# Virtana/accurate-aprilgroup-tracking

Hardware: AMD Instinct MI355X
Metric: frames/sec (LK+PnP) on 1280x720 dodeca stream (higher is better)
Workload: dtype u8/i64 (LK), f64 (PnP); 1 GPU; c2: 1 x 1280x720 stream(s) per GPU, 12 tags/48 corners, 3-level LK 21x21, iterative PnP with motion-model guess; streams_per_gpu=1, frames_resident=HBM ring 368 slots (323 MiB), parallelism=stream-per-GPU x1, RCCL all_gather of poses once per block

## Files before the change

### accurate_aprilgroup_tracking_amd/csrc/agt_pnp_body.h

```cpp
#pragma once
#include <type_traits>
#include <cstddef>
#include "agt_device.h"
#include "agt_kernels.h"

#ifdef AGT_PNP_STAMPS
__device__ unsigned long long agt_pnp_stamps[64];
#define PSTAMP(i) do { if (b == 0 && threadIdx.x == 0) agt_pnp_stamps[i] = __builtin_amdgcn_s_memtime(); } while (0)
#define PSTAMPM(i) do { int mk_; asm volatile("s_mov_b32 %0, %1" : "=s"(mk_) : "n"(0xbeef00 + (i))); PSTAMP(i); } while (0)
extern "C" int agt_debug_pnp_stamps(unsigned long long* host64)
{
    return (int)hipMemcpyFromSymbol(host64, HIP_SYMBOL(agt_pnp_stamps), sizeof(agt_pnp_stamps));
}
#else
#define PSTAMP(i)
#define PSTAMPM(i)
#endif

#pragma clang fp contract(fast)

namespace agt_pnp {

constexpr int NACC = 28;
constexpr int SLAB = 65;
constexpr int MAX_PPL = 4;

__device__ __forceinline__ void pnp_sync()
{
    __builtin_amdgcn_fence(__ATOMIC_RELEASE, "wavefront");
    __builtin_amdgcn_wave_barrier();
    __builtin_amdgcn_fence(__ATOMIC_ACQUIRE, "wavefront");
}

struct PnpShared {
    double part[NACC * SLAB];
    double tot[NACC + 4];
    double LL[144];
    double vec[48];
    unsigned long long tab[5 * AGT_MAX_GROUP];
    int seq;
    int late;
    int coop[2];
    AgtTrackState ts;
};

typedef __attribute__((address_space(3))) AgtTrackState AgtTrackStateLds;

template <int K, bool READBACK = true>
__device__ __forceinline__ void wave_reduce_slab(double (&vals)[K], PnpShared& sh, int lane)
{
    static_assert(K <= NACC, "the slab holds NACC rows");
    pnp_sync();
#pragma unroll
    for (int k = 0; k < K; k++) sh.part[k * SLAB + lane] = vals[k];
    pnp_sync();
    const int k = lane & 31, h = lane >> 5;
    double s = 0.0;
    if (k < K) {
        const double* p = &sh.part[k * SLAB + 32 * h];
#pragma unroll 8
        for (int i = 0; i < 32; i++) s += p[i];
    }
    s += __shfl_xor(s, 32);
    if (lane < K) sh.tot[lane] = s;
    pnp_sync();
    if (READBACK) {
#pragma unroll
        for (int i = 0; i < K; i++) vals[i] = sh.tot[i];
    }
}

__device__ __forceinline__ double dswap32(double a, double b, double& b_out)
{
    const auto lo = __builtin_amdgcn_permlane32_swap((unsigned)__double2loint(a), (unsigned)__double2loint(b), false, false);
    const auto hi = __builtin_amdgcn_permlane32_swap((unsigned)__double2hiint(a), (unsigned)__double2hiint(b), false, false);
    b_out = __hiloint2double((int)hi[1], (int)lo[1]);
    return __hiloint2double((int)hi[0], (int)lo[0]);
}
__device__ __forceinline__ double dswap16(double a, double b, double& b_out)
{
    const auto lo = __builtin_amdgcn_permlane16_swap((unsigned)__double2loint(a), (unsigned)__double2loint(b), false, false);
    const auto hi = __builtin_amdgcn_permlane16_swap((unsigned)__double2hiint(a), (unsigned)__double2hiint(b), false, false);
    b_out = __hiloint2double((int)hi[1], (int)lo[1]);
    return __hiloint2double((int)hi[0], (int)lo[0]);
}
template <int CTRL>
__device__ __forceinline__ double ddpp(double v)
{
    return __hiloint2double(agt_dpp_i32<CTRL>(__double2hiint(v)), agt_dpp_i32<CTRL>(__double2loint(v)));
}
template <int CTRL, int N>
__device__ __forceinline__ void bfly_stage(double (&v)[32], bool upper)
{
#pragma unroll
    for (int i = 0; i < N; i++) {
        const double a = v[i], b = v[i + N];
        const double keep = upper ? b : a, send = upper ? a : b;
// ... 255 lines not shown
        }
        const int slot = n_after - 1;
        for (int i = 0; i < 9; i++) ts->rot_vel[slot][i] = rot_vel[i];
        for (int i = 0; i < 3; i++) ts->tran_vel[slot][i] = tran_vel[i];
        ts->n_vel = n_after;
    }
    if (n_after < 2) return 0;
    double dv[3], tran_acc[3], rot_acc[9];
#pragma unroll
    for (int i = 0; i < 3; i++) dv[i] = old_tv[i] - tran_vel[i];
    mat3_tvec(rot_vel, dv, tran_acc);
    mat3_tmul(rot_vel, old_rv, rot_acc);
    const double sy = agt_sqrtp(rot_acc[0] * rot_acc[0] + rot_acc[3] * rot_acc[3]);
    const bool sing = sy < 1e-6;
    double ay, ax;
    if (lane == 0) { ay = sing ? -rot_acc[5] : rot_acc[7]; ax = sing ? rot_acc[4] : rot_acc[8]; }
    else if (lane == 1) { ay = -rot_acc[6]; ax = sy; }
    else { ay = sing ? 0.0 : rot_acc[3]; ax = sing ? 1.0 : rot_acc[0]; }
    double sn, cs;
    {
        const double r = agt_sqrtp(ax * ax + ay * ay);
        if (r > 0.0) {
            const double ir = agt_rcp(r), c = ax * ir, sv = ay * ir;
            if (c >= 0.0) { cs = agt_sqrtp(0.5 * (1.0 + c)); sn = sv * agt_rcp(2.0 * cs); }
            else { const double a = agt_sqrtp(0.5 * (1.0 - c)); sn = copysign(a, ay); cs = fabs(sv) * agt_rcp(2.0 * a); }
        } else { cs = 1.0; sn = 0.0; }
    }
    const double sx = lane_bcast(sn, 0), cx = lane_bcast(cs, 0);
    const double sy2 = lane_bcast(sn, 1), cy = lane_bcast(cs, 1);
    const double sz = lane_bcast(sn, 2), cz = lane_bcast(cs, 2);
    const double Rx[9] = { 1, 0, 0, 0, cx, -sx, 0, sx, cx };
    const double Ry[9] = { cy, 0, sy2, 0, 1, 0, -sy2, 0, cy };
    const double Rz[9] = { cz, -sz, 0, sz, cz, 0, 0, 0, 1 };
    double Tm[9], RA[9], M[9], Rpred[9], tp[3], tpred[3];
    agt_mat3_mul(Ry, Rx, Tm);
    agt_mat3_mul(Rz, Tm, RA);
    agt_mat3_mul(RA, rot_vel, M);
    agt_mat3_mul(M, Rp, Rpred);
#pragma unroll
    for (int i = 0; i < 3; i++) tp[i] = prev[3 + i];
#pragma unroll
    for (int i = 0; i < 3; i++)
        tpred[i] = (M[i * 3] * tp[0] + M[i * 3 + 1] * tp[1] + M[i * 3 + 2] * tp[2]) +
                   (RA[i * 3] * tran_vel[0] + RA[i * 3 + 1] * tran_vel[1] + RA[i * 3 + 2] * tran_vel[2] + 0.5 * tran_acc[i]);
    double rpred[3];
    agt_rodrigues_inv(Rpred, rpred);
    if (lane == 0) {
        for (int i = 0; i < 3; i++) { ts->guess[i] = rpred[i]; ts->guess[3 + i] = (double)(float)tpred[i]; }
        ts->guess_t_f32 = 1;
    }
    return 0;
}

struct PnpNoHook { __device__ __forceinline__ void operator()() const {} };

template <typename T, int PPL, typename Hook = PnpNoHook, bool LDS_STATE = false, int COOP = 1, bool OPAQUE = false, bool VIS = false, bool CONS = false>
__device__ __forceinline__ void pnp_body(const AgtPnpParams& P, int b, PnpShared& sh, const void* img_p, const uint8_t* mask_p,
                                         double* so_p, int extra_flags = 0, Hook before_state = Hook())
{
    using TS = typename std::conditional<LDS_STATE, AgtTrackStateLds, AgtTrackState>::type;
    static_assert(COOP == 1 || (PPL == 1 && COOP * 32 * 3 <= NACC * SLAB), "cooperating waves hold one point per lane; slabs live in sh.part");
    int tid_ = (int)threadIdx.x;
    if constexpr (OPAQUE) asm volatile("" : "+v"(tid_));
    const int lane = tid_ & (AGT_WAVE - 1);
    const int wave = COOP > 1 ? agt_uniform(tid_ >> 6) : 0;
    const bool master = wave == 0;
    const bool writer = lane == 0 && master;
    const int n = P.n;
    int slab_sel = 0;
    double* const tot = COOP > 1 ? &sh.part[2 * COOP * 32 + wave * 32] : sh.tot;
    auto coop_sum = [&](double v) -> double {
        if constexpr (COOP == 1) return v;
        else {
            double* slot = &sh.part[slab_sel * COOP * 32];
            if (lane == 0) slot[wave * 32] = v;
            __syncthreads();
            double s_ = slot[0];
#pragma unroll
            for (int w = 1; w < COOP; w++) s_ += slot[w * 32];
            slab_sel ^= 1;
            return s_;
        }
    };
    PSTAMP(0);
    AgtCamera cam;
    load_cam<T>(P.cam, cam);

    double X[PPL], Y[PPL], Z[PPL], mu_[PPL], mv_[PPL];
    bool use[PPL];
    const int hyp_T = CONS ? P.hyp_T : 0;
    const int hs = hyp_T ? b / hyp_T : b;
    const T* obj = reinterpret_cast<const T*>(P.obj) + (long)hs * P.obj_bstride + (hyp_T ? (long)(b - hs * hyp_T) * n * 3 : 0L);
    const T* img = reinterpret_cast<const T*>(img_p) + (long)b * n * 2;
    const uint8_t* mask = mask_p ? mask_p + (long)b * n : nullptr;
    const uint8_t* cons = (CONS && P.cons_inl) ? P.cons_inl + (long)b * n : nullptr;
    int cnt = 0;
#pragma unroll
    for (int q = 0; q < PPL; q++) {
        const int i = lane + (q * COOP + wave) * AGT_WAVE;
        use[q] = i < n && (!mask || mask[i] != 0) && (!cons || cons[i] != 0);
        X[q] = Y[q] = Z[q] = mu_[q] = mv_[q] = 0.0;
        if (use[q]) {
            X[q] = (double)obj[i * 3]; Y[q] = (double)obj[i * 3 + 1]; Z[q] = (double)obj[i * 3 + 2];
            mu_[q] = (double)img[i * 2]; mv_[q] = (double)img[i * 2 + 1];
            cnt++;
        }
    }
    if (P.seed_pts) {
        for (int i = lane + wave * AGT_WAVE; i < n; i += AGT_WAVE * COOP) {
            P.seed_pts[((long)b * n + i) * 2] = (float)img[i * 2]; P.seed_pts[((long)b * n + i) * 2 + 1] = (float)img[i * 2 + 1];
            P.seed_status[(long)b * n + i] = (!mask || mask[i] != 0) ? 1 : 0;
        }
    }
    if (P.tag_gate) {
        cnt = 0;
#pragma unroll
        for (int q = 0; q < PPL; q++) {
            int u = use[q] ? 1 : 0;
            u &= agt_dpp_i32<0xB1>(u);
            u &= agt_dpp_i32<0x4E>(u);
            use[q] = u != 0;
            if (!use[q]) X[q] = Y[q] = Z[q] = mu_[q] = mv_[q] = 0.0;
            cnt += u;
        }
    }
    const int n_used = (int)coop_sum((double)agt_wave_sum_i64(cnt));
    before_state();
    int flags = extra_flags;
    double param[6];
    TS* ts;
    if constexpr (LDS_STATE) ts = (TS*)&sh.ts;
    else ts = P.track ? P.track + b : nullptr;
    if (ts && (agt_uniform(ts->chain_fault) | (extra_flags & AGT_TRK_CHAIN_TIMEOUT))) {
        if (writer) {
            ts->chain_fault = 1; ts->frame++;
            if (P.fault) __hip_atomic_store(P.fault, 1, __ATOMIC_RELAXED, __HIP_MEMORY_SCOPE_SYSTEM);
            if (P.dense_pose) {
                for (int i = 0; i < AGT_DENSE_STRIDE; i++) P.dense_rec[(long)b * AGT_DENSE_STRIDE + i] = 0.0;
                P.dense_done[b] = 1;
            }
            if (so_p) {
                double* so = so_p + (long)b * AGT_STATE_STRIDE;
                for (int i = 0; i < AGT_STATE_STRIDE; i++) so[i] = 0.0;
                so[AGT_ST_NTRACK] = n_used; so[AGT_ST_FLAGS] = AGT_TRK_CHAIN_TIMEOUT;
            }
        }
        return;
    }
    bool use_guess = P.use_guess != 0;
    double unchanged_prev[6] = { 0, 0, 0, 0, 0, 0 };
    int had_guess = 0, guess_f32 = 0, prev_f32 = 0;
    if (ts) {
        had_guess = ts->has_guess; guess_f32 = ts->guess_t_f32; prev_f32 = ts->prev_t_f32;
        use_guess = had_guess && P.enhance_ape;
#pragma unroll
        for (int i = 0; i < 6; i++) { unchanged_prev[i] = ts->prev[i]; param[i] = ts->guess[i]; }
        static_assert(offsetof(AgtTrackState, tran_vel) - offsetof(AgtTrackState, rot_vel) == 18 * sizeof(double) &&
                      offsetof(AgtTrackState, prev_R) - offsetof(AgtTrackState, rot_vel) == 24 * sizeof(double), "state layout");
        if (had_guess && P.enhance_ape && lane < 33 && master) sh.vec[lane] = (&ts->rot_vel[0][0])[lane];
        if (n_used < P.min_points) {
            if (writer) {
                ts->has_guess = 0; ts->frame++;
                if (P.dense_pose) {
                    for (int i = 0; i < AGT_DENSE_STRIDE; i++) P.dense_rec[(long)b * AGT_DENSE_STRIDE + i] = 0.0;
                    P.dense_done[b] = 1;
                }
                if (so_p) {
                    double* so = so_p + (long)b * AGT_STATE_STRIDE;
                    for (int i = 0; i < AGT_STATE_STRIDE; i++) so[i] = 0.0;
                    so[AGT_ST_NTRACK] = n_used; so[AGT_ST_FLAGS] = AGT_PNP_TOO_FEW | flags;
                    if constexpr (CONS) { if (P.cons_votes) so[AGT_ST_NINLIER] = (double)P.cons_votes[b * 4 + 1]; }
                    if constexpr (CONS) { if (P.pred_hist) so[AGT_ST_FLOW] = P.pred_hist[(long)b * AGT_PRED_STRIDE + AGT_PRED_FLOW]; }
                }
            }
            return;
        }
    } else {
        const double* start = P.pose + (long)b * 6;
        if constexpr (CONS) {
            if (P.hyp_track) { use_guess = agt_uniform(P.hyp_track[hs].has_guess) && P.enhance_ape; start = P.hyp_track[hs].guess; }
            else if (P.hyp_pose) start = P.hyp_pose + (long)hs * 6;
        }
#pragma unroll
        for (int i = 0; i < 6; i++) param[i] = start[i];
    }

    const bool enough = use_guess ? n_used >= 3 : n_used >= 4;
    if (!enough) {
        if (writer && P.info) {
            P.info[b * 4 + AGT_INFO_OK] = 0; P.info[b * 4 + AGT_INFO_ITERS] = 0;
            P.info[b * 4 + AGT_INFO_NUSED] = n_used; P.info[b * 4 + AGT_INFO_FLAGS] = AGT_PNP_TOO_FEW;
        }
        if (writer && P.err) P.err[b] = 0.0;
        return;
    }

    if constexpr (COOP > 1) { if (!use_guess) return; }
    if constexpr (COOP == 1) if (!use_guess) {
        double c4[4] = { 0, 0, 0, 0 };
#pragma unroll
        for (int q = 0; q < PPL; q++) if (use[q]) { c4[0] += X[q]; c4[1] += Y[q]; c4[2] += Z[q]; }
        wave_reduce_slab<4>(c4, sh, lane);
        const double mcx = c4[0] / n_used, mcy = c4[1] / n_used, mcz = c4[2] / n_used;
        double m6[6] = { 0, 0, 0, 0, 0, 0 };
#pragma unroll
        for (int q = 0; q < PPL; q++) if (use[q]) {
            const double dx = X[q] - mcx, dy = Y[q] - mcy, dz = Z[q] - mcz;
            m6[0] += dx * dx; m6[1] += dx * dy; m6[2] += dx * dz; m6[3] += dy * dy; m6[4] += dy * dz; m6[5] += dz * dz;
        }
        wave_reduce_slab<6>(m6, sh, lane);
        const double MM[9] = { m6[0], m6[1], m6[2], m6[1], m6[3], m6[4], m6[2], m6[4], m6[5] };
        double Wm[3], Um[9], Vm[9];
        agt_svd3(MM, Wm, Um, Vm);
        if (Wm[2] / Wm[1] < 1e-3) {
            flags |= AGT_PNP_PLANAR;
            double Rt[9];
#pragma unroll
            for (int i = 0; i < 9; i++) Rt[i] = Vm[i];
            if (Vm[2] * Vm[2] + Vm[5] * Vm[5] < 1e-10) {
#pragma unroll
                for (int i = 0; i < 9; i++) Rt[i] = (i % 4 == 0) ? 1.0 : 0.0;
            }
            if (agt_det3(Rt) < 0) {
#pragma unroll
                for (int i = 0; i < 9; i++) Rt[i] = -Rt[i];
            }
            double Tt[3];
#pragma unroll
            for (int a = 0; a < 3; a++) Tt[a] = -(Rt[a * 3] * mcx + Rt[a * 3 + 1] * mcy + Rt[a * 3 + 2] * mcz);
            double px_[PPL], py_[PPL], nx_[PPL], ny_[PPL];
            double c8[8] = { 0, 0, 0, 0, 0, 0, 0, 0 };
#pragma unroll
            for (int q = 0; q < PPL; q++) {
                px_[q] = py_[q] = nx_[q] = ny_[q] = 0.0;
                if (use[q]) {
                    px_[q] = (double)(float)(Rt[0] * X[q] + Rt[1] * Y[q] + Rt[2] * Z[q] + Tt[0]);
                    py_[q] = (double)(float)(Rt[3] * X[q] + Rt[4] * Y[q] + Rt[5] * Z[q] + Tt[1]);
                    undistort5(cam, mu_[q], mv_[q], nx_[q], ny_[q]);
                    nx_[q] = (double)(float)nx_[q]; ny_[q] = (double)(float)ny_[q];
                    c8[0] += nx_[q]; c8[1] += ny_[q]; c8[2] += px_[q]; c8[3] += py_[q];
                }
            }
            wave_reduce_slab<8>(c8, sh, lane);
            const double cmx = c8[0] / n_used, cmy = c8[1] / n_used, cMx = c8[2] / n_used, cMy = c8[3] / n_used;
            double d8[8] = { 0, 0, 0, 0, 0, 0, 0, 0 };
#pragma unroll
            for (int q = 0; q < PPL; q++) if (use[q]) {
                d8[0] += fabs(nx_[q] - cmx); d8[1] += fabs(ny_[q] - cmy); d8[2] += fabs(px_[q] - cMx); d8[3] += fabs(py_[q] - cMy);
            }
            wave_reduce_slab<8>(d8, sh, lane);
// ... 168 lines not shown
                            lambda_h = lc = 1.0 / sh.vec[14];
                            nu *= 0.5;
                        }
                        lambda_h *= nu;
                    }
                    if (Sd < S) {
#pragma unroll
                        for (int i = 0; i < 8; i++) hx[i] = xd[i];
                        hom_eval(hx);
                        rinf = rinf_d;
                    }
                    it++;
                    double dinf = 0.0;
#pragma unroll
                    for (int i = 0; i < 8; i++) dinf = fmax(dinf, fabs(dd[i]));
                    if (!(it < 10 && dinf >= (double)FLT_EPSILON && rinf >= (double)FLT_EPSILON)) break;
                }
            }
            pnp_sync();
            if (lane == 0) {
                double h[9];
                for (int i = 0; i < 8; i++) h[i] = hx[i];
                h[8] = sh.vec[40];
                double Rm[9], tv[3];
                if (h_ok) {
                    const double h1n = sqrt(h[0] * h[0] + h[3] * h[3] + h[6] * h[6]);
                    const double h2n = sqrt(h[1] * h[1] + h[4] * h[4] + h[7] * h[7]);
                    const double s1 = 1. / fmax(h1n, DBL_EPSILON), s2 = 1. / fmax(h2n, DBL_EPSILON), s3 = 2. / fmax(h1n + h2n, DBL_EPSILON);
                    const double t3[3] = { h[2] * s3, h[5] * s3, h[8] * s3 };
                    h[0] *= s1; h[3] *= s1; h[6] *= s1;
                    h[1] *= s2; h[4] *= s2; h[7] *= s2;
                    h[2] = h[3] * h[7] - h[6] * h[4];
                    h[5] = h[6] * h[1] - h[0] * h[7];
                    h[8] = h[0] * h[4] - h[3] * h[1];
                    double rr[3], dummy[27];
                    agt_rodrigues_inv(h, rr);
                    agt_rodrigues<false>(rr, h, dummy);
                    for (int a = 0; a < 3; a++) tv[a] = h[a * 3] * Tt[0] + h[a * 3 + 1] * Tt[1] + h[a * 3 + 2] * Tt[2] + t3[a];
                    agt_mat3_mul(h, Rt, Rm);
                } else {
                    for (int i = 0; i < 9; i++) Rm[i] = (i % 4 == 0) ? 1.0 : 0.0;
                    tv[0] = tv[1] = tv[2] = 0.0;
                }
                double rv[3];
                agt_rodrigues_inv(Rm, rv);
                sh.vec[32] = rv[0]; sh.vec[33] = rv[1]; sh.vec[34] = rv[2];
                sh.vec[35] = tv[0]; sh.vec[36] = tv[1]; sh.vec[37] = tv[2];
            }
            pnp_sync();
#pragma unroll
            for (int i = 0; i < 6; i++) param[i] = sh.vec[32 + i];
        } else {
        if (n_used < 6) {
            if (lane == 0 && P.info) {
                P.info[b * 4 + AGT_INFO_OK] = 0; P.info[b * 4 + AGT_INFO_ITERS] = 0;
                P.info[b * 4 + AGT_INFO_NUSED] = n_used; P.info[b * 4 + AGT_INFO_FLAGS] = AGT_PNP_TOO_FEW;
            }
            if (lane == 0 && P.err) P.err[b] = 0.0;
            if (lane == 0 && ts) {
                ts->has_guess = 0; ts->frame++;
                if (P.dense_pose) {
                    for (int i = 0; i < AGT_DENSE_STRIDE; i++) P.dense_rec[(long)b * AGT_DENSE_STRIDE + i] = 0.0;
                    P.dense_done[b] = 1;
                }
                if (so_p) {
                    double* so = so_p + (long)b * AGT_STATE_STRIDE;
                    for (int i = 0; i < AGT_STATE_STRIDE; i++) so[i] = 0.0;
                    so[AGT_ST_NTRACK] = n_used; so[AGT_ST_FLAGS] = AGT_PNP_TOO_FEW | flags;
                    if constexpr (CONS) { if (P.cons_votes) so[AGT_ST_NINLIER] = (double)P.cons_votes[b * 4 + 1]; }
                    if constexpr (CONS) { if (P.pred_hist) so[AGT_ST_FLOW] = P.pred_hist[(long)b * AGT_PRED_STRIDE + AGT_PRED_FLOW]; }
                }
            }
            return;
        }
        double s0[10], sx[10], sy[10], sq[10];
#pragma unroll
        for (int i = 0; i < 10; i++) s0[i] = sx[i] = sy[i] = sq[i] = 0.0;
#pragma unroll
        for (int q = 0; q < PPL; q++) if (use[q]) {
            double xn, yn;
            undistort5(cam, mu_[q], mv_[q], xn, yn);
            const double x = -xn, y = -yn, w2 = x * x + y * y;
            const double pr[10] = { X[q] * X[q], X[q] * Y[q], X[q] * Z[q], X[q], Y[q] * Y[q], Y[q] * Z[q], Y[q], Z[q] * Z[q], Z[q], 1.0 };
#pragma unroll
            for (int i = 0; i < 10; i++) { s0[i] += pr[i]; sx[i] += x * pr[i]; sy[i] += y * pr[i]; sq[i] += w2 * pr[i]; }
        }
        wave_reduce_slab<10>(s0, sh, lane);
        wave_reduce_slab<10>(sx, sh, lane);
        wave_reduce_slab<10>(sy, sh, lane);
        wave_reduce_slab<10>(sq, sh, lane);
        pnp_sync();
        if (lane == 0) {
            const int ui[4][4] = { { 0, 1, 2, 3 }, { 1, 4, 5, 6 }, { 2, 5, 7, 8 }, { 3, 6, 8, 9 } };
            for (int a = 0; a < 4; a++)
                for (int c = 0; c < 4; c++) {
                    const int u = ui[a][c];
                    sh.LL[a * 12 + c] = s0[u];           sh.LL[a * 12 + 4 + c] = 0.0;          sh.LL[a * 12 + 8 + c] = sx[u];
                    sh.LL[(4 + a) * 12 + c] = 0.0;       sh.LL[(4 + a) * 12 + 4 + c] = s0[u];  sh.LL[(4 + a) * 12 + 8 + c] = sy[u];
                    sh.LL[(8 + a) * 12 + c] = sx[u];     sh.LL[(8 + a) * 12 + 4 + c] = sy[u];  sh.LL[(8 + a) * 12 + 8 + c] = sq[u];
                }
        }
        pnp_sync();
        smallest_eigvec_wave<12>(sh.LL, sh.vec, lane);
        if (lane == 0) {
            double* v = sh.vec;
            double RR[9] = { v[0], v[1], v[2], v[4], v[5], v[6], v[8], v[9], v[10] };
            double tt[3] = { v[3], v[7], v[11] };
            if (agt_det3(RR) < 0) {
                for (int i = 0; i < 9; i++) RR[i] = -RR[i];
                for (int i = 0; i < 3; i++) tt[i] = -tt[i];
            }
            double sc = 0;
            for (int i = 0; i < 9; i++) sc += RR[i] * RR[i];
            sc = sqrt(sc);
            double Wr[3], U[9], Vt[9], Rm[9];
            agt_svd3(RR, Wr, U, Vt);
            agt_mat3_mul(U, Vt, Rm);
            double nr = 0;
            for (int i = 0; i < 9; i++) nr += Rm[i] * Rm[i];
            nr = sqrt(nr);
            double rv[3];
            agt_rodrigues_inv(Rm, rv);
            sh.vec[32] = rv[0]; sh.vec[33] = rv[1]; sh.vec[34] = rv[2];
            sh.vec[35] = tt[0] * nr / sc; sh.vec[36] = tt[1] * nr / sc; sh.vec[37] = tt[2] * nr / sc;
        }
        pnp_sync();
// ... 74 lines not shown
#pragma unroll
            for (int i = 0; i < 6; i++) JtErr[i] = tot[21 + i];
            return tot[27];
        }
        double e2 = 0.0;
#pragma unroll
        for (int q = 0; q < PPL; q++) if (PPL > 1 || use[q]) {
            double u, v;
            agt_project<false, D>(cam, R, G, param + 3, X[q], Y[q], Z[q], u, v, nullptr, nullptr);
            const double m = (PPL > 1 && !use[q]) ? 0.0 : 1.0;
            const double ex = (u - mu_[q]) * m, ey = (v - mv_[q]) * m;
            rex[q] = ex; rey[q] = ey;
            e2 += ex * ex + ey * ey;
        }
        return coop_sum(wave_sum_f64(e2));
    };
    auto evaluate = [&](int mode) -> double {
        return has_dist ? evaluate_t(mode, std::true_type{}) : evaluate_t(mode, std::false_type{});
    };
    auto commit_candidate = [&]() {
#pragma unroll
        for (int i = 0; i < 21; i++) JtJ[i] = tot[i];
#pragma unroll
        for (int i = 0; i < 6; i++) JtErr[i] = tot[21 + i];
    };
    auto residuals_same_rotation = [&](auto DIST) {
        constexpr bool D = decltype(DIST)::value;
#pragma unroll
        for (int q = 0; q < PPL; q++) if (use[q]) {
            double u, v;
            agt_project<false, D>(cam, Rlast, nullptr, param + 3, X[q], Y[q], Z[q], u, v, nullptr, nullptr);
            rex[q] = u - mu_[q]; rey[q] = v - mv_[q];
        }
    };

    auto step = [&]() {
        double A[36], dx[6];
        int idx = 0;
#pragma unroll
        for (int a = 0; a < 6; a++)
#pragma unroll
            for (int c = a; c < 6; c++) { A[a * 6 + c] = JtJ[idx]; A[c * 6 + a] = JtJ[idx]; idx++; }
#pragma unroll
        for (int a = 0; a < 6; a++) A[a * 7] *= 1.0 + lambda;
        if (!agt_solve6(A, JtErr, dx)) {
            flags |= AGT_PNP_SINGULAR;
#pragma unroll
            for (int a = 0; a < 6; a++) dx[a] = 0.0;
        }
#pragma unroll
        for (int a = 0; a < 6; a++) param[a] = prevParam[a] - dx[a];
    };

    PSTAMP(1);
    double e2 = evaluate(1);
    PSTAMP(2);
    for (;;) {
#pragma unroll
        for (int i = 0; i < 6; i++) prevParam[i] = param[i];
        if (iters == 0) prevErrNorm = sqrt(e2);
        double rel = 0.0, e2cand = 0.0;
        bool last = false;
        for (;;) {
            PSTAMP(8 + iters * 4 + 0);
            step();
            PSTAMP(8 + iters * 4 + 1);
            double dn = 0.0, pn = 0.0;
#pragma unroll
            for (int i = 0; i < 6; i++) { const double d = param[i] - prevParam[i]; dn += d * d; pn += prevParam[i] * prevParam[i]; }
            rel = sqrt(dn) / (sqrt(pn) + DBL_EPSILON);
            last = iters + 1 >= max_iter || rel < epsilon;
            e2cand = evaluate(last ? 0 : 2);
            errNorm = sqrt(e2cand);
            PSTAMP(8 + iters * 4 + 2);
            if (errNorm > prevErrNorm) { ++lambdaLg10; lambda *= 10.0; if (lambdaLg10 <= 16) continue; }
            break;
        }
        if (lambdaLg10 - 1 >= -16) { lambdaLg10 -= 1; lambda *= 0.1; } else { lambdaLg10 = -16; lambda = 1e-16; }
        ++iters;
        if (last) break;
        prevErrNorm = errNorm;
        commit_candidate();
        e2 = e2cand;
        PSTAMP(8 + (iters - 1) * 4 + 3);
    }
    PSTAMP(3);

    const bool tvec_f32 = ts && use_guess && guess_f32;
    if (tvec_f32) {
#pragma unroll
        for (int i = 3; i < 6; i++) param[i] = (double)(float)param[i];
    }

    double esum = 0.0;
    {
        if (tvec_f32) { if (has_dist) residuals_same_rotation(std::true_type{}); else residuals_same_rotation(std::false_type{}); }
#pragma unroll
        for (int q = 0; q < PPL; q++) if (use[q]) esum += sqrt(rex[q] * rex[q] + rey[q] * rey[q]);
        esum = coop_sum(wave_sum_f64(esum)) / n_used;
    }
    PSTAMP(4);
    if (!master) return;
    if (ts) {
        const bool accepted = esum < P.gate_px;
        int tflags = flags;
        if (writer && use_guess) {
            for (int i = 0; i < 6; i++) ts->guess[i] = param[i];
        }
        if (accepted && had_guess && P.enhance_ape)
            tflags |= motion_model_update(ts, lane, param, tvec_f32, unchanged_prev, prev_f32 != 0, Rlast, sh.vec);
        if (writer) {
            if (accepted) {
                if (!had_guess || !P.enhance_ape) {
                    for (int i = 0; i < 6; i++) ts->guess[i] = param[i];
                    ts->guess_t_f32 = 0; ts->has_guess = 1;
                }
                if (!(tflags & AGT_TRK_ZERO_VELOCITY)) {
                    for (int i = 0; i < 6; i++) ts->prev[i] = param[i];
                    for (int i = 0; i < 9; i++) ts->prev_R[i] = Rlast[i];
                    ts->prev_t_f32 = tvec_f32 ? 1 : 0; ts->has_prev = 1;
                }
            } else {
                ts->has_guess = 0;
            }
            ts->frame++;
            PSTAMP(5);
            if (P.dense_pose) {
                double* rc = P.dense_rec + (long)b * AGT_DENSE_STRIDE;
                for (int i = 0; i < 6; i++) { P.dense_pose[(long)b * 6 + i] = param[i]; rc[i] = param[i]; }
                for (int i = 6; i < AGT_DENSE_STRIDE; i++) rc[i] = 0.0;
                P.dense_done[b] = accepted ? 0 : 1;
            }
            if (so_p) {
                double* so = so_p + (long)b * AGT_STATE_STRIDE;
                for (int i = 0; i < 6; i++) so[i] = param[i];
                so[AGT_ST_OK] = accepted ? 1.0 : 0.0; so[AGT_ST_ERR] = esum; so[AGT_ST_NTRACK] = n_used;
                so[AGT_ST_ITERS] = iters; so[AGT_ST_GUESS] = use_guess ? 1.0 : 0.0; so[AGT_ST_FLAGS] = tflags;
                so[AGT_ST_TVEC_F32] = tvec_f32 ? 1.0 : 0.0;
                for (int i = AGT_ST_TVEC_F32 + 1; i < AGT_STATE_STRIDE; i++) so[i] = 0.0;
                if constexpr (CONS) { if (P.cons_votes) so[AGT_ST_NINLIER] = (double)P.cons_votes[b * 4 + 1]; }
                if constexpr (CONS) { if (P.pred_hist) so[AGT_ST_FLOW] = P.pred_hist[(long)b * AGT_PRED_STRIDE + AGT_PRED_FLOW]; }
            }
            if constexpr (CONS) {
                if (P.pred_hist) {
                    double* h = P.pred_hist + (long)b * AGT_PRED_STRIDE + AGT_PRED_LAST;
                    for (int i = 0; i < 6; i++) h[i] = param[i];
                    h[6] = accepted ? 1.0 : 0.0;
                }
            }
        }
        if (accepted && P.reproject && P.corners_rw) {
            double R[9], G[9];
            agt_rodrigues<false>(param, R, G);
            float* cw = P.corners_rw + (long)b * n * 2;
            const int cpt = VIS ? P.vis_cpt : 0;
            unsigned long long seen = ~0ull;
            if (cpt > 0) {
                double cs;
                const bool vis = lane < n / cpt && agt_tag_visible(obj + (long)lane * cpt * 3, cpt, R, param + 3, (double)P.vis_facing, P.vis_cos_max, cs);
                seen = __ballot(vis);
                if (writer && so_p) so_p[(long)b * AGT_STATE_STRIDE + AGT_ST_NVISIBLE] = (double)__popcll(seen);
            }
            for (int i = lane; i < n; i += AGT_WAVE) {
                double u, v;
                agt_project<false>(cam, R, G, param + 3, (double)obj[i * 3], (double)obj[i * 3 + 1], (double)obj[i * 3 + 2],
                                   u, v, nullptr, nullptr);
                cw[i * 2] = (float)u; cw[i * 2 + 1] = (float)v;
                if (P.status_rw) P.status_rw[(long)b * n + i] = cpt > 0 ? (uint8_t)((seen >> (i / cpt)) & 1) : 1;
            }
        }
        return;
    }
    if (writer) {
#pragma unroll
        for (int i = 0; i < 6; i++) P.pose[(long)b * 6 + i] = param[i];
        if (P.info) {
            P.info[b * 4 + AGT_INFO_OK] = 1; P.info[b * 4 + AGT_INFO_ITERS] = iters;
            P.info[b * 4 + AGT_INFO_NUSED] = n_used; P.info[b * 4 + AGT_INFO_FLAGS] = flags;
        }
        if (P.err) P.err[b] = esum;
    }
}

}

#pragma clang fp contract(off)
```

### accurate_aprilgroup_tracking_amd/csrc/agt_step.hip

```cpp
#undef AGT_LK_STAMPS
#undef AGT_PNP_STAMPS
#include "agt_step_args.h"
#include "agt_knobs.h"

#ifdef AGT_STEP_STAMPS
__device__ unsigned long long agt_step_stamps[16];
#define SSTAMP_SET(i) do { if (threadIdx.x == 0) agt_step_stamps[i] = __builtin_amdgcn_s_memtime(); } while (0)
#define SSTAMP_MAX(i) do { if (threadIdx.x == 0) atomicMax(&agt_step_stamps[i], (unsigned long long)__builtin_amdgcn_s_memtime()); } while (0)
#define SSTAMP_MIN(i) do { if (threadIdx.x == 0) atomicMin(&agt_step_stamps[i], (unsigned long long)__builtin_amdgcn_s_memtime()); } while (0)
extern "C" int agt_debug_step_stamps(unsigned long long* host16, int reset)
{
    int rc = (int)hipMemcpyFromSymbol(host16, HIP_SYMBOL(agt_step_stamps), sizeof(agt_step_stamps));
    if (reset) {
        unsigned long long z[16];
        for (int i = 0; i < 16; i++) z[i] = (i == 6) ? ~0ull : 0ull;
        rc |= (int)hipMemcpyToSymbol(HIP_SYMBOL(agt_step_stamps), z, sizeof(z));
    }
    return rc;
}
__device__ unsigned long long agt_role_stamps[AGT_MAX_GROUP * 4];
#define RSTAMP(k, i) do { if (blk == 0 && lane == 0) agt_role_stamps[(k) * 4 + (i)] = __builtin_amdgcn_s_memtime(); } while (0)
extern "C" int agt_debug_role_stamps(unsigned long long* host) { return (int)hipMemcpyFromSymbol(host, HIP_SYMBOL(agt_role_stamps), sizeof(agt_role_stamps)); }
#else
#define SSTAMP_SET(i)
#define SSTAMP_MAX(i)
#define SSTAMP_MIN(i)
#define RSTAMP(k, i)
#endif


typedef unsigned long long __attribute__((may_alias)) agt_word_t;
__device__ __forceinline__ void agt_copy_words_to_lds(void* dst_lds, const void* src, int n8, int t, int stride)
{
    for (int i = t; i < n8; i += stride) static_cast<agt_word_t*>(dst_lds)[i] = static_cast<const agt_word_t*>(src)[i];
}
typedef unsigned int __attribute__((may_alias)) agt_halfword_t;
__device__ __forceinline__ void agt_copy_halfwords_to_lds(void* dst_lds, const void* src, int n4, int t, int stride)
{
    for (int i = t; i < n4; i += stride) static_cast<agt_halfword_t*>(dst_lds)[i] = static_cast<const agt_halfword_t*>(src)[i];
}
__device__ __forceinline__ bool agt_ptr_plausible(unsigned long long p) { return (p >> 47) == 0; }
template <int NLEV>
__device__ __forceinline__ bool lk_table_bad(const agt_lk::LkFrameIo<NLEV>& io, int max_level)
{
    unsigned long long acc = (unsigned long long)io.next_pts | (unsigned long long)io.status | (unsigned long long)io.done;
    bool null_img = io.next_pts == nullptr || io.status == nullptr;
#pragma unroll
    for (int l = 0; l < NLEV; l++)
        if (l <= max_level) {
            acc |= (unsigned long long)io.imgI[l] | (unsigned long long)io.imgJ[l];
            null_img = null_img || io.imgI[l] == nullptr || io.imgJ[l] == nullptr;
        }
    return agt_uniform((int)(null_img || !agt_ptr_plausible(acc))) != 0;
}

hipError_t agt_launch_pnp_group_coop(hipStream_t stream, const AgtStepParams& P, const AgtStepTables& T);
hipError_t agt_launch_step_deep(hipStream_t stream, const AgtStepParams& P, const AgtStepTables& T, int blocks, size_t lds);

namespace {

template <int WIN, int NW, int NLEV, bool XCD_MAP = false>
__device__ __forceinline__ void lk_role(const AgtStepParams& S, const AgtStepTables& T, KParams KS, KTables KT, int blk, uint8_t* lds)
{
    static_assert(NW == 4, "one corner per workgroup of four waves");
    if constexpr (XCD_MAP) blk = agt_xcd_order(blk, (int)gridDim.x, KS->xshift);
    const long corner = blk;
    if (corner >= (long)S.lk.n * S.lk_B) return;
    const int b = (int)(corner / S.lk.n), pt = (int)(corner - (long)b * S.lk.n);
    constexpr size_t LKB = sizeof(AgtLkTables);
    const size_t per = lk_role_lds<WIN, NW, NLEV>(S.lk.max_level + 1);
    uint8_t* my = lds;
    AgtLkTables* tab = reinterpret_cast<AgtLkTables*>(my + per - LKB);
    {
        static_assert(sizeof(AgtLkTables) % 8 == 0, "table copy: 8-byte words");
        const int tid = (int)threadIdx.x;
        if (S.lk_nf > 1) agt_copy_words_to_lds(tab, (const void*)(const __attribute__((address_space(4))) void*)&KT->lk, (int)(LKB / 8), tid, AGT_WAVE * NW);
    }
    if constexpr (WIN == 21 && NW == 4) {
        if (S.lk.flags == 0 && S.lk.err == nullptr) {
            auto frame = [&](int k) {
// ... 39 lines not shown
        if (io.bad) return;
        agt_lk::lk_body<WIN, NW, NLEV>(&KS->lk, pt, b, my, io, px, py, pst);
    }
}

template <bool ROLL2>
__device__ __forceinline__ void pyr_role(KParams KS, KTables KT, int blk, int base, uint8_t* lds)
{
#pragma unroll
    for (int s = 0; s < AGT_MAX_LEVELS - 1; s++) {
        const int n = KS->n_pyr[s];
        if (blk < n) {
            AgtPyrArgs A;
            A.src = nullptr; A.dst = nullptr; A.strip_rows = 0; A.topdown = 0;
            A.spitch = KS->pyr[s].spitch; A.sbatch = KS->pyr[s].sbatch; A.dpitch = KS->pyr[s].dpitch; A.dbatch = KS->pyr[s].dbatch;
            A.sw = KS->pyr[s].sw; A.sh = KS->pyr[s].sh; A.dw = KS->pyr[s].dw; A.dh = KS->pyr[s].dh;
            A.gx = KS->pyr[s].gx; A.gy = KS->pyr[s].gy; A.B = KS->pyr[s].B; A.strip_rows = KS->pyr[s].strip_rows;
            const int xs = ROLL2 ? KS->xshift : 3, xm = (1 << xs) - 1;
            const int j = (blk + base) & xm;
            int tile = (blk - ((j - base) & xm)) >> xs;
            for (int q = 0; q < j; q++) tile += (n - ((q - base) & xm) + xm) >> xs;
            const int per_img = agt_pyr_blocks(A);
            const int bz = tile / per_img, r = tile - bz * per_img;
            const int by = r / A.gx, bx = r - by * A.gx;
            const int fr = bz / A.B, st = bz - fr * A.B;
            if (s == 0 && KS->pyr_fused) {
                AgtPyrArgs A1;
                A1.src = nullptr; A1.dst = nullptr; A1.strip_rows = 0;
                A1.spitch = KS->pyr[1].spitch; A1.sbatch = KS->pyr[1].sbatch; A1.dpitch = KS->pyr[1].dpitch; A1.dbatch = KS->pyr[1].dbatch;
                A1.sw = KS->pyr[1].sw; A1.sh = KS->pyr[1].sh; A1.dw = KS->pyr[1].dw; A1.dh = KS->pyr[1].dh;
                A1.gx = A.gx; A1.gy = A.gy; A1.B = A.B;
                if (ROLL2 && agt_pyr_rolling(A)) {
                    A.topdown = KS->pyr[0].topdown;
                    agt_pyr4::pyr_roll2_body(A, A1, bx, KT->pyr_src[0][fr] + (long)st * A.sbatch, KT->pyr_dst[0][fr] + (long)st * A.dbatch,
                                             KT->pyr_dst[1][fr] + (long)st * A1.dbatch);
                    return;
                }
                agt_pyr2::pyr_down2_body(A, A1, bx, by, KT->pyr_src[0][fr] + (long)st * A.sbatch, KT->pyr_dst[0][fr] + (long)st * A.dbatch,
                                         KT->pyr_dst[1][fr] + (long)st * A1.dbatch, lds);
                return;
            }
            if (agt_pyr_rolling(A)) {
                agt_pyr3::pyr_roll_body(A, bx, KT->pyr_src[s][fr] + (long)st * A.sbatch, KT->pyr_dst[s][fr] + (long)st * A.dbatch);
                return;
            }
            agt_pyr::pyr_down_body(A, bx, by, KT->pyr_src[s][fr] + (long)st * A.sbatch, KT->pyr_dst[s][fr] + (long)st * A.dbatch, lds);
            return;
        }
        blk -= n;
        base += n;
    }
}

template <int PPL, int NWV = 1>
__device__ __forceinline__ void pnp_role(const AgtStepParams& S, const AgtStepTables& T, KTables KT, int blk, agt_pnp::PnpShared& sh, int wave = 0)
{
    static_assert(sizeof(AgtPnpTables) == 40 * AGT_MAX_GROUP && sizeof(sh.tab) == sizeof(AgtPnpTables), "table layout");
    static_assert(sizeof(AgtTrackState) % 8 == 0 && sizeof(AgtTrackState) / 8 <= AGT_WAVE, "state copy: one double per lane");
    const int lane = (int)(threadIdx.x & (AGT_WAVE - 1));
    if (NWV == 1) {
        if (S.pnp_nf > 1) agt_copy_words_to_lds(sh.tab, (const void*)(const __attribute__((address_space(4))) void*)&KT->pnp, (int)(sizeof(AgtPnpTables) / 8), lane, AGT_WAVE);
        agt_copy_words_to_lds(&sh.ts, S.pnp.track + blk, (int)(sizeof(AgtTrackState) / 8), lane, AGT_WAVE);
        __builtin_amdgcn_fence(__ATOMIC_RELEASE, "workgroup"); __builtin_amdgcn_wave_barrier(); __builtin_amdgcn_fence(__ATOMIC_ACQUIRE, "workgroup");
    }
    int late = 0;
    for (int k = wave; k < S.pnp_nf; k += NWV) {
        const void* img = T.pnp.img[0]; const uint8_t* mask = T.pnp.mask[0]; double* so = T.pnp.so[0];
        const unsigned* wait = T.pnp.wait[0]; unsigned target = (unsigned)T.pnp.target[0];
        RSTAMP(k, 0);
        if (k) {
            if (NWV == 1) { asm volatile("s_waitcnt lgkmcnt(0)" ::: "memory"); __builtin_amdgcn_wave_barrier(); }
            unsigned long long t_img = sh.tab[k], t_mask = sh.tab[AGT_MAX_GROUP + k], t_so = sh.tab[2 * AGT_MAX_GROUP + k];
            unsigned long long t_wait = sh.tab[3 * AGT_MAX_GROUP + k];
            target = (unsigned)sh.tab[4 * AGT_MAX_GROUP + k];
            if (!agt_uniform((int)(t_img != 0 && agt_ptr_plausible(t_img | t_mask | t_so | t_wait)))) {
                late = 1;
                t_img = (unsigned long long)T.pnp.img[0]; t_mask = 0; t_wait = 0;
                if (!agt_ptr_plausible(t_so)) t_so = 0;
            }
            img = (const void*)t_img; mask = (const uint8_t*)t_mask; so = (double*)t_so; wait = (const unsigned*)t_wait;
        }
        if (wait) {
            if (!late) {
                int timed_out = 0;
                if (lane == 0) {
                    const int* fault = &S.pnp.track[blk].chain_fault;
                    unsigned polls = 0;
                    while ((int)(__hip_atomic_load(wait + blk, __ATOMIC_RELAXED, __HIP_MEMORY_SCOPE_AGENT) - target) < 0) {
                        __builtin_amdgcn_s_sleep(4);
                        if ((NWV > 1 && *(volatile int*)&sh.late) || ++polls > AGT_CHAIN_POLLS ||
                            ((polls & 15) == 1 && __hip_atomic_load(fault, __ATOMIC_RELAXED, __HIP_MEMORY_SCOPE_AGENT))) { timed_out = 1; break; }
                    }
                    if (timed_out && NWV > 1) *(volatile int*)&sh.late = 1;
                }
                late = agt_uniform(__shfl(timed_out, 0));
            }
            __builtin_amdgcn_fence(__ATOMIC_ACQUIRE, "agent");
        }
        RSTAMP(k, 1);
        auto before_state = [&]() {
            RSTAMP(k, 1);
            if (NWV > 1) {
                while (agt_uniform(*(volatile int*)&sh.seq) < k) __builtin_amdgcn_s_sleep(1);
                asm volatile("" ::: "memory");
            }
            RSTAMP(k, 2);
        };
        agt_pnp::pnp_body<float, PPL, decltype(before_state), true>(S.pnp, blk, sh, img, mask, so, late ? AGT_TRK_CHAIN_TIMEOUT : 0, before_state);
        asm volatile("s_waitcnt lgkmcnt(0)" ::: "memory");
        RSTAMP(k, 3);
        if (k == S.pnp_nf - 1 && lane < (int)(sizeof(AgtTrackState) / 8))
            reinterpret_cast<agt_word_t*>(S.pnp.track + blk)[lane] = reinterpret_cast<const agt_word_t*>(&sh.ts)[lane];
        if (NWV > 1) {
            if (lane == 0) *(volatile int*)&sh.seq = k + 1;
        }
        if (S.pnp.host_seq && blk == 0 && k == S.pnp_nf - 1) agt_host_seq_store(S.pnp.host_seq, S.pnp.host_seq_base + (unsigned long long)k, lane == 0);
    }
}

__device__ __forceinline__ void pnp_role_coop(const AgtStepParams& S, const AgtStepTables& T, KTables KT, int blk, agt_pnp::PnpShared& sh)
{
    const int tid = (int)threadIdx.x, wave = tid >> 6;
    int late = 0;
#pragma nounroll
    for (int k = 0; k < S.pnp_nf; k++) {
        __syncthreads();
        const void* img = (const void*)KT->pnp.img[k]; const uint8_t* mask = KT->pnp.mask[k]; double* so = KT->pnp.so[k];
        const unsigned* wait = KT->pnp.wait[k]; const unsigned target = (unsigned)KT->pnp.target[k];
        if (wait) {
            if (!late) {
                if (tid == 0) {
                    const int* fault = &S.pnp.track[blk].chain_fault;
                    unsigned polls = 0;
                    int timed_out = 0;
                    while ((int)(__hip_atomic_load(wait + blk, __ATOMIC_RELAXED, __HIP_MEMORY_SCOPE_AGENT) - target) < 0) {
                        __builtin_amdgcn_s_sleep(4);
                        if (++polls > AGT_CHAIN_POLLS || ((polls & 15) == 1 && __hip_atomic_load(fault, __ATOMIC_RELAXED, __HIP_MEMORY_SCOPE_AGENT))) { timed_out = 1; break; }
                    }
                    *(volatile int*)&sh.late = timed_out;
                }
                __syncthreads();
                late = agt_uniform(*(volatile int*)&sh.late);
            }
        }
        __builtin_amdgcn_fence(__ATOMIC_ACQUIRE, "agent");
        const bool guess = agt_uniform(__hip_atomic_load(&S.pnp.track[blk].has_guess, __ATOMIC_RELAXED, __HIP_MEMORY_SCOPE_AGENT)) != 0 && S.pnp.enhance_ape;
        __syncthreads();
        const int xf = late ? AGT_TRK_CHAIN_TIMEOUT : 0;
        KParams KF = kernarg_params();
        int bk = blk;
        asm volatile("" : "+s"(KF), "+s"(bk));
        const AgtPnpParams& PF = *(const AgtPnpParams*)&KF->pnp;
        if (guess) agt_pnp::pnp_body<float, 1, agt_pnp::PnpNoHook, false, PNP_COOP, true>(PF, bk, sh, img, mask, so, xf);
        else if (wave == 0) agt_pnp::pnp_body<float, agt_pnp::MAX_PPL, agt_pnp::PnpNoHook, false, 1, true>(PF, bk, sh, img, mask, so, xf);
        if (wave == 0) {
            __builtin_amdgcn_fence(__ATOMIC_RELEASE, "agent");
            if (S.pnp.host_seq && blk == 0 && k == S.pnp_nf - 1) agt_host_seq_store(S.pnp.host_seq, S.pnp.host_seq_base + (unsigned long long)k, tid == 0);
        }
    }
}

template <int WIN, int NW, int NLEV, bool PNP, int OCC>
__global__ __launch_bounds__(STEP_THREADS) __attribute__((amdgpu_waves_per_eu(OCC))) void step_kernel(const AgtStepParams S, const AgtStepTables T)
{
    extern __shared__ __attribute__((aligned(16))) uint8_t lds[];
    KParams KS = kernarg_params();
    KTables KT = kernarg_tables();
    int blk = blockIdx.x;
    SSTAMP_MIN(6);
    if (blk < S.n_lk) {
        if (blk == 0) SSTAMP_SET(2);
        lk_role<WIN, NW, NLEV>(S, T, KS, KT, blk, lds);
        if (blk == 0) SSTAMP_SET(3);
        SSTAMP_MAX(4);
        return;
    }
    blk -= S.n_lk;
    if (PNP && blk < S.n_pnp) {
        agt_pnp::PnpShared& sh = *reinterpret_cast<agt_pnp::PnpShared*>(lds);
        agt_copy_halfwords_to_lds(sh.tab, (const void*)(const __attribute__((address_space(4))) void*)&KT->pnp, (int)(sizeof(AgtPnpTables) / 4), (int)threadIdx.x, STEP_THREADS);
        if (threadIdx.x == 0) { sh.seq = 0; sh.late = 0; }
        agt_copy_words_to_lds(&sh.ts, S.pnp.track + blk, (int)(sizeof(AgtTrackState) / 8), (int)threadIdx.x, STEP_THREADS);
        __syncthreads();
        const int wave = (int)(threadIdx.x / AGT_WAVE);
        if (wave >= 2) return;
        if (blk == 0 && wave == 0) SSTAMP_SET(0);
        pnp_role<1, 2>(S, T, KT, blk, sh, wave);
        if (blk == 0 && wave == 0) SSTAMP_SET(1);
        return;
    }
    if (PNP) blk -= S.n_pnp;
    pyr_role<false>(KS, KT, blk, (PNP ? S.n_pnp : 0) + S.n_lk, lds);
    SSTAMP_MAX(5);
}

template <int WIN, int NW, int NLEV, int OCC>
__global__ __launch_bounds__(AGT_WAVE * NW) __attribute__((amdgpu_waves_per_eu(OCC))) void lk_group_kernel(const AgtStepParams S, const AgtStepTables T)
{
    extern __shared__ __attribute__((aligned(16))) uint8_t lds[];
    lk_role<WIN, NW, NLEV, true>(S, T, kernarg_params(), kernarg_tables(), blockIdx.x, lds);
}

#ifndef AGT_STEP_NOLICM_TU
__global__ __launch_bounds__(agt_pyr::NT) void pyr_group_kernel(const AgtStepParams S, const AgtStepTables T)
{
    extern __shared__ __attribute__((aligned(16))) uint8_t lds[];
    pyr_role<true>(kernarg_params(), kernarg_tables(), blockIdx.x, 0, lds);
}
#endif

template <int PPL>
__global__ __launch_bounds__(AGT_WAVE) void pnp_group_kernel(const AgtStepParams S, const AgtStepTables T)
{
    __shared__ agt_pnp::PnpShared sh;
    pnp_role<PPL>(S, T, kernarg_tables(), blockIdx.x, sh);
}

#ifdef AGT_STEP_NOLICM_TU
__global__ __launch_bounds__(AGT_WAVE * PNP_COOP) void pnp_group_coop_kernel(const AgtStepParams S, const AgtStepTables T)
{
    __shared__ agt_pnp::PnpShared sh;
    pnp_role_coop(S, T, kernarg_tables(), blockIdx.x, sh);
}
#endif

}

#ifdef AGT_STEP_NOLICM_TU
hipError_t agt_launch_pnp_group_coop(hipStream_t stream, const AgtStepParams& P, const AgtStepTables& T)
{
    hipLaunchKernelGGL(pnp_group_coop_kernel, dim3(P.n_pnp), dim3(AGT_WAVE * PNP_COOP), 0, stream, P, T);
    return hipGetLastError();
}

// ... 66 lines not shown
```

Before: 78210 frames/s.

## Speculatively hand over PnP state before the acceptance gate, with verdict-based redo

In the two-wave PnP role, each wave now publishes the updated tracking state, which releases the next frame's wave, before computing the residual-based acceptance check. The previous state is snapshotted and restored if the gate rejects. A per-frame verdict slot in LDS lets the following wave detect a rejected predecessor and recompute its frame. This shortens the serial dependency chain between consecutive frames. The cost is extra polling, LDS snapshot traffic, and occasional redundant recomputation after a rejection.

```diff
diff --git a/accurate_aprilgroup_tracking_amd/csrc/agt_pnp_body.h b/accurate_aprilgroup_tracking_amd/csrc/agt_pnp_body.h
--- a/accurate_aprilgroup_tracking_amd/csrc/agt_pnp_body.h
+++ b/accurate_aprilgroup_tracking_amd/csrc/agt_pnp_body.h
@@ -42,7 +42,9 @@
     int late;
     int coop[2];
     AgtTrackState ts;
+    int verdict[2];
 };
+typedef unsigned long long __attribute__((may_alias)) PnpStateWord;
 
 typedef __attribute__((address_space(3))) AgtTrackState AgtTrackStateLds;
 
@@ -404,14 +406,16 @@
     return 0;
 }
 
-struct PnpNoHook { __device__ __forceinline__ void operator()() const {} };
-
-template <typename T, int PPL, typename Hook = PnpNoHook, bool LDS_STATE = false, int COOP = 1, bool OPAQUE = false, bool VIS = false, bool CONS = false>
-__device__ __forceinline__ void pnp_body(const AgtPnpParams& P, int b, PnpShared& sh, const void* img_p, const uint8_t* mask_p,
-                                         double* so_p, int extra_flags = 0, Hook before_state = Hook())
+struct PnpNoHook { __device__ __forceinline__ void operator()() const {} __device__ __forceinline__ void handed_over() const {} __device__ __forceinline__ void verdict_stored() const {} };
+
+template <typename T, int PPL, typename Hook = PnpNoHook, bool LDS_STATE = false, int COOP = 1, bool OPAQUE = false, bool VIS = false, bool CONS = false,
+          bool SPEC = false>
+__device__ __forceinline__ int pnp_body(const AgtPnpParams& P, int b, PnpShared& sh, const void* img_p, const uint8_t* mask_p,
+                                        double* so_p, int extra_flags = 0, Hook before_state = Hook(), int spec_k = 0, int spec_prev = 0)
 {
     using TS = typename std::conditional<LDS_STATE, AgtTrackStateLds, AgtTrackState>::type;
     static_assert(COOP == 1 || (PPL == 1 && COOP * 32 * 3 <= NACC * SLAB), "cooperating waves hold one point per lane; slabs live in sh.part");
+    static_assert(!SPEC || (LDS_STATE && COOP == 1 && !VIS && !CONS), "speculation: the one-wave body on the LDS state of the fused step");
     int tid_ = (int)threadIdx.x;
     if constexpr (OPAQUE) asm volatile("" : "+v"(tid_));
     const int lane = tid_ & (AGT_WAVE - 1);
@@ -483,7 +487,26 @@
     TS* ts;
     if constexpr (LDS_STATE) ts = (TS*)&sh.ts;
     else ts = P.track ? P.track + b : nullptr;
+    auto prev_frame_stands = [&]() -> bool {
+        int v = 1;
+        if constexpr (SPEC) {
+            if (spec_prev) {
+                while (abs(v = agt_uniform(*(volatile int*)&sh.verdict[(spec_prev - 1) & 1])) != spec_prev) __builtin_amdgcn_s_sleep(1);
+                asm volatile("" ::: "memory");
+            }
+        }
+        return v > 0;
+    };
+    auto leave_unsolved = [&]() {
+        if constexpr (SPEC) {
+            asm volatile("s_waitcnt lgkmcnt(0)" ::: "memory");
+            before_state.handed_over();
+            if (lane == 0) { *(volatile int*)&sh.seq = spec_k + 1; *(volatile int*)&sh.verdict[spec_k & 1] = spec_k + 1; }
+            before_state.verdict_stored();
+        }
+    };
     if (ts && (agt_uniform(ts->chain_fault) | (extra_flags & AGT_TRK_CHAIN_TIMEOUT))) {
+        if constexpr (SPEC) { if (!prev_frame_stands()) return 1; }
         if (writer) {
             ts->chain_fault = 1; ts->frame++;
             if (P.fault) __hip_atomic_store(P.fault, 1, __ATOMIC_RELAXED, __HIP_MEMORY_SCOPE_SYSTEM);
@@ -497,7 +520,8 @@
                 so[AGT_ST_NTRACK] = n_used; so[AGT_ST_FLAGS] = AGT_TRK_CHAIN_TIMEOUT;
             }
         }
-        return;
+        if constexpr (SPEC) leave_unsolved();
+        return 0;
     }
     bool use_guess = P.use_guess != 0;
     double unchanged_prev[6] = { 0, 0, 0, 0, 0, 0 };
@@ -511,6 +535,7 @@
                       offsetof(AgtTrackState, prev_R) - offsetof(AgtTrackState, rot_vel) == 24 * sizeof(double), "state layout");
         if (had_guess && P.enhance_ape && lane < 33 && master) sh.vec[lane] = (&ts->rot_vel[0][0])[lane];
         if (n_used < P.min_points) {
+            if constexpr (SPEC) { if (!prev_frame_stands()) return 1; }
             if (writer) {
                 ts->has_guess = 0; ts->frame++;
                 if (P.dense_pose) {
@@ -525,7 +550,8 @@
                     if constexpr (CONS) { if (P.pred_hist) so[AGT_ST_FLOW] = P.pred_hist[(long)b * AGT_PRED_STRIDE + AGT_PRED_FLOW]; }
                 }
             }
-            return;
+            if constexpr (SPEC) leave_unsolved();
+            return 0;
         }
     } else {
         const double* start = P.pose + (long)b * 6;
@@ -539,15 +565,17 @@
 
     const bool enough = use_guess ? n_used >= 3 : n_used >= 4;
     if (!enough) {
+        if constexpr (SPEC) { if (!prev_frame_stands()) return 1; }
         if (writer && P.info) {
             P.info[b * 4 + AGT_INFO_OK] = 0; P.info[b * 4 + AGT_INFO_ITERS] = 0;
             P.info[b * 4 + AGT_INFO_NUSED] = n_used; P.info[b * 4 + AGT_INFO_FLAGS] = AGT_PNP_TOO_FEW;
         }
         if (writer && P.err) P.err[b] = 0.0;
-        return;
-    }
-
-    if constexpr (COOP > 1) { if (!use_guess) return; }
+        if constexpr (SPEC) leave_unsolved();
+        return 0;
+    }
+
+    if constexpr (COOP > 1) { if (!use_guess) return 0; }
     if constexpr (COOP == 1) if (!use_guess) {
         double c4[4] = { 0, 0, 0, 0 };
 #pragma unroll
@@ -822,6 +850,7 @@
             for (int i = 0; i < 6; i++) param[i] = sh.vec[32 + i];
         } else {
         if (n_used < 6) {
+            if constexpr (SPEC) { if (!prev_frame_stands()) return 1; }
             if (lane == 0 && P.info) {
                 P.info[b * 4 + AGT_INFO_OK] = 0; P.info[b * 4 + AGT_INFO_ITERS] = 0;
                 P.info[b * 4 + AGT_INFO_NUSED] = n_used; P.info[b * 4 + AGT_INFO_FLAGS] = AGT_PNP_TOO_FEW;
@@ -841,7 +870,8 @@
                     if constexpr (CONS) { if (P.pred_hist) so[AGT_ST_FLOW] = P.pred_hist[(long)b * AGT_PRED_STRIDE + AGT_PRED_FLOW]; }
                 }
             }
-            return;
+            if constexpr (SPEC) leave_unsolved();
+            return 0;
         }
         double s0[10], sx[10], sy[10], sq[10];
 #pragma unroll
@@ -1022,6 +1052,8 @@
         for (int a = 0; a < 6; a++) param[a] = prevParam[a] - dx[a];
     };
 
+    int spec_pv = spec_prev;
+    PnpStateWord spec_keep = 0ull;
     PSTAMP(1);
     double e2 = evaluate(1);
     PSTAMP(2);
@@ -1040,6 +1072,12 @@
             for (int i = 0; i < 6; i++) { const double d = param[i] - prevParam[i]; dn += d * d; pn += prevParam[i] * prevParam[i]; }
             rel = sqrt(dn) / (sqrt(pn) + DBL_EPSILON);
             last = iters + 1 >= max_iter || rel < epsilon;
+            if constexpr (SPEC) {
+                if (last) {
+                    if (spec_prev) spec_pv = *(volatile int*)&sh.verdict[(spec_prev - 1) & 1];
+                    spec_keep = lane < (int)(sizeof(AgtTrackState) / 8) ? reinterpret_cast<volatile PnpStateWord*>(&sh.ts)[lane] : 0ull;
+                }
+            }
             e2cand = evaluate(last ? 0 : 2);
             errNorm = sqrt(e2cand);
             PSTAMP(8 + iters * 4 + 2);
@@ -1063,6 +1101,76 @@
     }
 
     double esum = 0.0;
+    if constexpr (SPEC) {
+        constexpr int NW8 = (int)(sizeof(AgtTrackState) / 8);
+        volatile PnpStateWord* tsw = reinterpret_cast<volatile PnpStateWord*>(&sh.ts);
+        int pv = spec_pv;
+        PnpStateWord keep = spec_keep;
+        const bool mm = had_guess && P.enhance_ape;
+        while (abs(agt_uniform(pv)) != spec_prev) {
+            __builtin_amdgcn_s_sleep(1);
+            pv = *(volatile int*)&sh.verdict[(spec_prev - 1) & 1];
+            keep = lane < NW8 ? tsw[lane] : 0ull;
+        }
+        asm volatile("" ::: "memory");
+        if (agt_uniform(pv) < 0) return 1;
+        int mflags = 0;
+        if (writer && use_guess) {
+            for (int i = 0; i < 6; i++) ts->guess[i] = param[i];
+        }
+        if (mm) mflags = motion_model_update(ts, lane, param, tvec_f32, unchanged_prev, prev_f32 != 0, Rlast, sh.vec);
+        if (writer) {
+            if (!mm) {
+                for (int i = 0; i < 6; i++) ts->guess[i] = param[i];
+                ts->guess_t_f32 = 0; ts->has_guess = 1;
+            }
+            if (!(mflags & AGT_TRK_ZERO_VELOCITY)) {
+                for (int i = 0; i < 6; i++) ts->prev[i] = param[i];
+                for (int i = 0; i < 9; i++) ts->prev_R[i] = Rlast[i];
+                ts->prev_t_f32 = tvec_f32 ? 1 : 0; ts->has_prev = 1;
+            }
+        }
+        asm volatile("s_waitcnt lgkmcnt(0)" ::: "memory");
+        before_state.handed_over();
+        if (lane == 0) *(volatile int*)&sh.seq = spec_k + 1;
+        asm volatile("" ::: "memory");
+        if (tvec_f32) { if (has_dist) residuals_same_rotation(std::true_type{}); else residuals_same_rotation(std::false_type{}); }
+#pragma unroll
+        for (int q = 0; q < PPL; q++) if (use[q]) esum += sqrt(rex[q] * rex[q] + rey[q] * rey[q]);
+        esum = wave_sum_f64(esum) / n_used;
+        PSTAMP(4);
+        const bool accepted = esum < P.gate_px;
+        if (!accepted) {
+            if (lane < NW8) tsw[lane] = keep;
+            asm volatile("" ::: "memory");
+            if (writer) {
+                if (use_guess) { for (int i = 0; i < 6; i++) ts->guess[i] = param[i]; }
+                ts->has_guess = 0;
+            }
+        }
+        if (writer) {
+            ts->frame++;
+            PSTAMP(5);
+            if (P.dense_pose) {
+                double* rc = P.dense_rec + (long)b * AGT_DENSE_STRIDE;
+                for (int i = 0; i < 6; i++) { P.dense_pose[(long)b * 6 + i] = param[i]; rc[i] = param[i]; }
+                for (int i = 6; i < AGT_DENSE_STRIDE; i++) rc[i] = 0.0;
+                P.dense_done[b] = accepted ? 0 : 1;
+            }
+            if (so_p) {
+                double* so = so_p + (long)b * AGT_STATE_STRIDE;
+                for (int i = 0; i < 6; i++) so[i] = param[i];
+                so[AGT_ST_OK] = accepted ? 1.0 : 0.0; so[AGT_ST_ERR] = esum; so[AGT_ST_NTRACK] = n_used;
+                so[AGT_ST_ITERS] = iters; so[AGT_ST_GUESS] = use_guess ? 1.0 : 0.0; so[AGT_ST_FLAGS] = accepted ? (flags | mflags) : flags;
+                so[AGT_ST_TVEC_F32] = tvec_f32 ? 1.0 : 0.0;
+                for (int i = AGT_ST_TVEC_F32 + 1; i < AGT_STATE_STRIDE; i++) so[i] = 0.0;
+            }
+        }
+        asm volatile("s_waitcnt lgkmcnt(0)" ::: "memory");
+        if (lane == 0) *(volatile int*)&sh.verdict[spec_k & 1] = accepted ? spec_k + 1 : -(spec_k + 1);
+        before_state.verdict_stored();
+        return 0;
+    }
     {
         if (tvec_f32) { if (has_dist) residuals_same_rotation(std::true_type{}); else residuals_same_rotation(std::false_type{}); }
 #pragma unroll
@@ -1070,7 +1178,7 @@
         esum = coop_sum(wave_sum_f64(esum)) / n_used;
     }
     PSTAMP(4);
-    if (!master) return;
+    if (!master) return 0;
     if (ts) {
         const bool accepted = esum < P.gate_px;
         int tflags = flags;
@@ -1139,7 +1247,7 @@
                 if (P.status_rw) P.status_rw[(long)b * n + i] = cpt > 0 ? (uint8_t)((seen >> (i / cpt)) & 1) : 1;
             }
         }
-        return;
+        return 0;
     }
     if (writer) {
 #pragma unroll
@@ -1150,6 +1258,7 @@
         }
         if (P.err) P.err[b] = esum;
     }
+    return 0;
 }
 
 }
diff --git a/accurate_aprilgroup_tracking_amd/csrc/agt_step.hip b/accurate_aprilgroup_tracking_amd/csrc/agt_step.hip
--- a/accurate_aprilgroup_tracking_amd/csrc/agt_step.hip
+++ b/accurate_aprilgroup_tracking_amd/csrc/agt_step.hip
@@ -18,14 +18,16 @@
     }
     return rc;
 }
-__device__ unsigned long long agt_role_stamps[AGT_MAX_GROUP * 4];
+__device__ unsigned long long agt_role_stamps[AGT_MAX_GROUP * 5];
 #define RSTAMP(k, i) do { if (blk == 0 && lane == 0) agt_role_stamps[(k) * 4 + (i)] = __builtin_amdgcn_s_memtime(); } while (0)
+#define VSTAMP(k) do { if (blk == 0 && lane == 0) agt_role_stamps[AGT_MAX_GROUP * 4 + (k)] = __builtin_amdgcn_s_memtime(); } while (0)
 extern "C" int agt_debug_role_stamps(unsigned long long* host) { return (int)hipMemcpyFromSymbol(host, HIP_SYMBOL(agt_role_stamps), sizeof(agt_role_stamps)); }
 #else
 #define SSTAMP_SET(i)
 #define SSTAMP_MAX(i)
 #define SSTAMP_MIN(i)
 #define RSTAMP(k, i)
+#define VSTAMP(k)
 #endif
 
 
@@ -171,6 +173,13 @@
     }
 }
 
+template <typename Wait>
+struct PnpSpecHook {
+    const Wait& wait; int k, blk, lane;
+    __device__ __forceinline__ void operator()() const { wait(); }
+    __device__ __forceinline__ void handed_over() const { RSTAMP(k, 3); }
+    __device__ __forceinline__ void verdict_stored() const { VSTAMP(k); }
+};
 template <int PPL, int NWV = 1>
 __device__ __forceinline__ void pnp_role(const AgtStepParams& S, const AgtStepTables& T, KTables KT, int blk, agt_pnp::PnpShared& sh, int wave = 0)
 {
@@ -182,7 +191,7 @@
         agt_copy_words_to_lds(&sh.ts, S.pnp.track + blk, (int)(sizeof(AgtTrackState) / 8), lane, AGT_WAVE);
         __builtin_amdgcn_fence(__ATOMIC_RELEASE, "workgroup"); __builtin_amdgcn_wave_barrier(); __builtin_amdgcn_fence(__ATOMIC_ACQUIRE, "workgroup");
     }
-    int late = 0;
+    int late = 0, again = 0;
     for (int k = wave; k < S.pnp_nf; k += NWV) {
         const void* img = T.pnp.img[0]; const uint8_t* mask = T.pnp.mask[0]; double* so = T.pnp.so[0];
         const unsigned* wait = T.pnp.wait[0]; unsigned target = (unsigned)T.pnp.target[0];
@@ -225,14 +234,18 @@
             }
             RSTAMP(k, 2);
         };
-        agt_pnp::pnp_body<float, PPL, decltype(before_state), true>(S.pnp, blk, sh, img, mask, so, late ? AGT_TRK_CHAIN_TIMEOUT : 0, before_state);
+        if constexpr (NWV > 1) {
+            const PnpSpecHook<decltype(before_state)> hook{ before_state, k, blk, lane };
+            const int redo = agt_pnp::pnp_body<float, PPL, decltype(hook), true, 1, false, false, false, true>(
+                S.pnp, blk, sh, img, mask, so, late ? AGT_TRK_CHAIN_TIMEOUT : 0, hook, k, (k > 0 && !again) ? k : 0);
+            again = agt_uniform(redo);
+            if (again) { k -= NWV; continue; }
+        } else
+            agt_pnp::pnp_body<float, PPL, decltype(before_state), true>(S.pnp, blk, sh, img, mask, so, late ? AGT_TRK_CHAIN_TIMEOUT : 0, before_state);
         asm volatile("s_waitcnt lgkmcnt(0)" ::: "memory");
-        RSTAMP(k, 3);
+        if (NWV == 1) { RSTAMP(k, 3); }
         if (k == S.pnp_nf - 1 && lane < (int)(sizeof(AgtTrackState) / 8))
             reinterpret_cast<agt_word_t*>(S.pnp.track + blk)[lane] = reinterpret_cast<const agt_word_t*>(&sh.ts)[lane];
-        if (NWV > 1) {
-            if (lane == 0) *(volatile int*)&sh.seq = k + 1;
-        }
         if (S.pnp.host_seq && blk == 0 && k == S.pnp_nf - 1) agt_host_seq_store(S.pnp.host_seq, S.pnp.host_seq_base + (unsigned long long)k, lane == 0);
     }
 }
@@ -298,7 +311,7 @@
     if (PNP && blk < S.n_pnp) {
         agt_pnp::PnpShared& sh = *reinterpret_cast<agt_pnp::PnpShared*>(lds);
         agt_copy_halfwords_to_lds(sh.tab, (const void*)(const __attribute__((address_space(4))) void*)&KT->pnp, (int)(sizeof(AgtPnpTables) / 4), (int)threadIdx.x, STEP_THREADS);
-        if (threadIdx.x == 0) { sh.seq = 0; sh.late = 0; }
+        if (threadIdx.x == 0) { sh.seq = 0; sh.late = 0; sh.verdict[0] = 0; sh.verdict[1] = 0; }
         agt_copy_words_to_lds(&sh.ts, S.pnp.track + blk, (int)(sizeof(AgtTrackState) / 8), (int)threadIdx.x, STEP_THREADS);
         __syncthreads();
         const int wave = (int)(threadIdx.x / AGT_WAVE);
```

Measured after the change: 78370 frames/s (median of 6 runs). No clear change (+0.2%).
